# KrishnaswamyLab/MELD

Hardware: AMD Instinct MI355X
Metric: cells/sec through MELD.fit_transform (kNN+Chebyshev) (higher is better)
Workload: dtype f64

## Files before the change

### meld_amd/csrc/knn16.hip

```cpp
#include "common.hpp"
#include "k16_rows.hpp"

#include <hip/hip_fp16.h>

#include <algorithm>

namespace meld {

constexpr int K16_TS = 64;
constexpr int K16_BQ = 256;
constexpr int K16_THREADS = 256;
constexpr int K16_NWAVE = K16_THREADS / 64;
constexpr int K16_SLACK = 128;
constexpr int K16_CAPMAX = K16_ROW_CAPMAX;
constexpr int K16_BOUNDS_THREADS = 1024;
constexpr int K16_SLOTS = K16_CAPMAX / 64;
constexpr int K16_DMAX = 16 * 9 - 3;

constexpr int K16_SPLIT_DA = 13;
__host__ __device__ inline void k16_slot(int c, int d, int dA, int* coord, int* piece) {
  *coord = -1;
  *piece = -1;
  if (dA == 0) {
    if (c < d) *coord = c;
// ... 523 lines not shown
#pragma unroll
      for (int kb = 0; kb < KB; ++kb) {
        __builtin_amdgcn_sched_group_barrier(0x008, 1, 0);
        __builtin_amdgcn_sched_group_barrier(0x002, VALU_PER_MFMA, 0);
        __builtin_amdgcn_sched_group_barrier(0x008, 1, 0);
        __builtin_amdgcn_sched_group_barrier(0x002, VALU_PER_MFMA, 0);
        if (kb + A_AHEAD < KB) __builtin_amdgcn_sched_group_barrier(0x100, 1, 0);
      }
    }
  };
  auto segment = [&](const _Float16* tile, int sub, f32x16& n0, f32x16& n1, const f32x16& c0, const f32x16& c1, int ref_base, bool issue,
                     bool fresh) __attribute__((always_inline)) {
    if (issue) mfma_block(tile, sub, n0, n1);
    float m0, m1;
    vote(c0, c1, m0, m1);
    if (issue) asm volatile("" : "+v"(m0), "+v"(m1));
    const bool hit = m0 < thrp[0] || m1 < thrp[1];
    if (issue) pipeline_order();
    if (fresh && __any(hit)) {
      unsigned t0s = tm_now();
      select(c0, c1, m0, m1, ref_base);
      if (STATS) {
        const unsigned d = tm_now() - t0s;
        tm_sel += d;
        tm_mark += d;
      }
    }
  };

  auto next_step = [&](int after, int par_, bool* live) __attribute__((always_inline)) {
    if (!my_lb) {
      *live = true;
      return after + 1;
    }
    unsigned long long any = lds_union(par_) & win_rem;
    if (__builtin_expect(any == 0, 0)) {
      while (any == 0 && win_base + 64 < n_scan) {
        load_window(win_base + 64);
        my_live = __ballot(win_lb <= wmax + prune_margin);
        if (lane == 0) lds_wlive[2][wave] = my_live;
        __syncthreads();
        any = lds_union(2) & win_rem;
        __syncthreads();
      }
      K16_COLD_REGION_END();
    }
    if (any == 0) {
      *live = false;
      return n_scan;
    }
    const int i = (int)__ffsll((long long)any) - 1;
    *live = (my_live >> i) & 1ull;
    win_rem &= ~((2ull << i) - 1ull);
    return win_base + i;
  };

  int n_done = 0;
  auto ee_tile = [&](const _Float16* tile_r, int t) __attribute__((always_inline)) {
    const f16x8* a8 = reinterpret_cast<const f16x8*>(tile_r) + jq;
    const f16x8 aA = a8[h * K16_TS], aB = a8[32 + h * K16_TS];
    const float tA0 = thrp[0] + ee_c[0], tA1 = thrp[1] + ee_c[1];
#pragma unroll
    for (int sub = 0; sub < 2; ++sub) {
#pragma unroll
      for (int r = 0; r < 16; ++r) accA0[r] = accA1[r] = 0.0f;
      accA0 = __builtin_amdgcn_mfma_f32_32x32x16_f16(sub ? aB : aA, bhi[0][0], accA0, 0, 0, 0);
      accA1 = __builtin_amdgcn_mfma_f32_32x32x16_f16(sub ? aB : aA, bhi[1][0], accA1, 0, 0, 0);
      if (__any(min16(accA0) < tA0 || min16(accA1) < tA1)) {
        const f16x8* as = a8 + sub * 32;
#pragma unroll
        for (int kb = 1; kb < KB; ++kb) {
          const f16x8 ahi = as[(kb * 2 + h) * K16_TS];
          accA0 = __builtin_amdgcn_mfma_f32_32x32x16_f16(ahi, bhi[0][kb], accA0, 0, 0, 0);
          accA1 = __builtin_amdgcn_mfma_f32_32x32x16_f16(ahi, bhi[1][kb], accA1, 0, 0, 0);
        }
        const float m0 = min16(accA0), m1 = min16(accA1);
        if (__any(m0 < thrp[0] || m1 < thrp[1])) {
          const unsigned t0s = tm_now();
          select(accA0, accA1, m0, m1, t * K16_TS + 32 * sub + 4 * h);
          if (STATS) {
            const unsigned dsel = tm_now() - t0s;
            tm_sel += dsel;
            tm_mark += dsel;
          }
        }
        ++st_go;
      }
    }
    ++n_done;
  };
  int s_cur = 0;
  int par = 0;
  int it = 0;
  bool live_cur = true;
  bool pend = false;
  unsigned e_pref = 0u;
  int t_cur = tile_of(0);
  bool live_next = true;
  int s_next = next_step(0, 0, &live_next);
  int t_next = s_next < n_scan ? tile_of(s_next) : t_cur;
  if constexpr (LIST) {
    const unsigned e0 = list_entry(0), e1 = list_entry(1);
    e_pref = list_entry(2);
    t_cur = (int)(e0 & 0xFFFFFFu);
    live_cur = entry_live(e0);
    s_next = 1;
    t_next = s_next < n_scan ? (int)(e1 & 0xFFFFFFu) : t_cur;
    live_next = entry_live(e1);
  }
  if constexpr (!PAIR) {
    if (s_next < n_scan) {
      K16_LOAD(__builtin_amdgcn_readfirstlane(t_next), (unsigned)TILE_LDS_BYTES);
      K16_STAGED_BUT_LAST();
    } else {
      K16_STAGED();
    }
    K16_TILE_BARRIER();
  }
  unsigned rd_b = 0u, nx_b = (unsigned)TILE_LDS_BYTES, wr_b = 2u * (unsigned)TILE_LDS_BYTES;
  auto scan_step = [&]() __attribute__((always_inline)) {
    const int t = t_cur;
    const _Float16* tile_r = reinterpret_cast<const _Float16*>(reinterpret_cast<const char*>(lds_ring) + rd_b);
    const bool tm_live = live_cur;
    unsigned e_far = 0u;
    if constexpr (LIST) e_far = list_entry(s_next + 2);
    if (EE && live_cur) {
      ee_tile(tile_r, t);
    } else if (live_cur) {
      segment(tile_r, 0, accA0, accA1, accB0, accB1, refB, true, pend);
      segment(tile_r, 1, accB0, accB1, accA0, accA1, t * K16_TS + 4 * h, true, true);
      refB = t * K16_TS + 32 + 4 * h;
      pend = true;
      ++n_done;
    } else if (pend) {
      segment(nullptr, 0, accA0, accA1, accB0, accB1, refB, false, true);
      pend = false;
    }

    if (tm_live) tm_lap(tm_seg); else tm_lap(tm_idle);
    if (batch_every > 0 && (it & (batch_every - 1)) == batch_every - 1) {
      const int limit = ksel + K16_COLD(batch_slack);
      unsigned long long todo = 0;
#pragma unroll
      for (int g = 0; g < 2; ++g) {
        const int cg = g ? cnt[1] : cnt[0];
        const int tot = cg + __shfl_xor(cg, 32, 64);
        todo |= (__ballot(tot > limit) & 0xffffffffull) << (32 * g);
      }
      if (todo) {
        while (todo) {
          const int j = __ffsll((long long)todo) - 1;
          todo &= todo - 1;
          squeeze(j >> 5, j & 31);
          if (STATS) ++st_sq;
        }
        refresh_wmax();
        K16_COLD_REGION_END();
      }
    }

    bool live_nn = true;
    int s_nn, t_nn;
    if constexpr (LIST) {
      s_nn = min(s_next + 1, n_scan);
      t_nn = s_nn < n_scan ? (int)(e_pref & 0xFFFFFFu) : t_next;
      live_nn = entry_live(e_pref);
      e_pref = e_far;
    } else {
      s_nn = s_next < n_scan ? next_step(s_next, par, &live_nn) : n_scan;
      t_nn = s_nn < n_scan ? tile_of(s_nn) : t_next;
    }

    if (s_nn < n_scan) {
      K16_LOAD(__builtin_amdgcn_readfirstlane(t_nn), wr_b);
      tm_lap(tm_tail);
      K16_STAGED_BUT_LAST();
    } else {
      tm_lap(tm_tail);
      K16_STAGED();
    }
    tm_lap(tm_dma);
    if (my_lb) {
      my_live = __ballot(win_lb <= wmax + prune_margin);
      if (lane == 0) lds_wlive[par ^ 1][wave] = my_live;
    }
    tm_lap(tm_tail);
    K16_TILE_BARRIER();
    tm_lap(tm_bar);
    s_cur = s_next;
    t_cur = t_next;
    live_cur = live_next;
    s_next = s_nn;
    t_next = t_nn;
    live_next = live_nn;
    par ^= 1;
    ++it;
    const unsigned free_b = rd_b;
    rd_b = nx_b;
    nx_b = wr_b;
    wr_b = free_b;
  };
  tm_mark = tm_now();
  if constexpr (PAIR) {
    constexpr unsigned PB = 2u * (unsigned)TILE_LDS_BYTES;
    const int n_pairs = (n_scan + 1) >> 1;
    unsigned c0 = list_entry(0), c1 = list_entry(1), x0 = list_entry(2), x1 = list_entry(3);
    if (n_scan > 0) K16_LOAD(__builtin_amdgcn_readfirstlane((int)(c0 & 0xFFFFFFu)), 0u);
    if (n_scan > 1) K16_LOAD(__builtin_amdgcn_readfirstlane((int)(c1 & 0xFFFFFFu)), (unsigned)TILE_LDS_BYTES);
    K16_STAGED();
    K16_TILE_BARRIER();
    for (int p = 0; p < n_pairs; ++p) {
      const unsigned buf = (p & 1) ? PB : 0u, other = PB - buf;
      const unsigned f0 = list_entry(2 * p + 4), f1 = list_entry(2 * p + 5);
      if (2 * p + 2 < n_scan) K16_LOAD(__builtin_amdgcn_readfirstlane((int)(x0 & 0xFFFFFFu)), other);
      if (2 * p + 3 < n_scan) K16_LOAD(__builtin_amdgcn_readfirstlane((int)(x1 & 0xFFFFFFu)), other + (unsigned)TILE_LDS_BYTES);
      tm_lap(tm_tail);
      const char* ring = reinterpret_cast<const char*>(lds_ring);
      const bool live0 = entry_live(c0), live1 = 2 * p + 1 < n_scan && entry_live(c1);
      if (live0) ee_tile(reinterpret_cast<const _Float16*>(ring + buf), (int)(c0 & 0xFFFFFFu));
      if (live1) ee_tile(reinterpret_cast<const _Float16*>(ring + buf + TILE_LDS_BYTES), (int)(c1 & 0xFFFFFFu));
      if (live0 || live1) tm_lap(tm_seg); else tm_lap(tm_idle);
      if (batch_every > 0 && (p & (batch_every / 2 - 1)) == batch_every / 2 - 1) {
        const int limit = ksel + K16_COLD(batch_slack);
        unsigned long long todo = 0;
#pragma unroll
        for (int g = 0; g < 2; ++g) {
          const int cg = g ? cnt[1] : cnt[0];
          const int tot = cg + __shfl_xor(cg, 32, 64);
          todo |= (__ballot(tot > limit) & 0xffffffffull) << (32 * g);
        }
        while (todo) {
          const int j = __ffsll((long long)todo) - 1;
          todo &= todo - 1;
          squeeze(j >> 5, j & 31);
          if (STATS) ++st_sq;
        }
      }
      tm_lap(tm_tail);
      K16_STAGED();
      tm_lap(tm_dma);
      K16_TILE_BARRIER();
      tm_lap(tm_bar);
      c0 = x0;
      c1 = x1;
      x0 = f0;
      x1 = f1;
      ++it;
    }
  }
  while (!PAIR && s_cur < n_scan) scan_step();
  if (pend) segment(nullptr, 0, accA0, accA1, accB0, accB1, refB, false, true);
  {
    unsigned long long* tiles_done = K16_COLD(tiles_done);
    if (tiles_done && lane == 0) {
      atomicAdd(tiles_done, (unsigned long long)n_done);
      if (EE && K16_COLD(count_go)) atomicAdd(tiles_done + 1, (unsigned long long)st_go);
    }
  }

  unsigned long long* stats = STATS ? K16_COLD(stats) : nullptr;
  if (STATS && stats) {
    unsigned a = st_app;
#pragma unroll
    for (int off = 32; off > 0; off >>= 1) a += __shfl_xor(a, off, 64);
    if (lane == 0) {
      atomicAdd(stats + 0, (unsigned long long)(2 * n_done));
      atomicAdd(stats + 1, (unsigned long long)st_slow);
      atomicAdd(stats + 2, (unsigned long long)a);
      atomicAdd(stats + 3, (unsigned long long)st_sq);
      const int it_tiles = PAIR ? n_scan : it;
      if (wave == 0) atomicAdd(stats + 4, (unsigned long long)it_tiles);
      atomicAdd(stats + 5, (unsigned long long)tm_seg);
      atomicAdd(stats + 6, (unsigned long long)tm_sel);
      atomicAdd(stats + 7, (unsigned long long)tm_tail);
      atomicAdd(stats + 8, (unsigned long long)tm_dma);
      atomicAdd(stats + 9, (unsigned long long)tm_bar);
      atomicAdd(stats + 10, (unsigned long long)tm_idle);
      atomicAdd(stats + 11, (unsigned long long)it_tiles);
      if (EE) atomicAdd(stats + 12, (unsigned long long)st_go);
    }
  }
  const float out_scale = K16_COLD(scale_info)[1];
  float* cand_thr = K16_COLD(cand_thr);
  int* cand_cnt = K16_COLD(cand_cnt);
  if (cand_thr && h == 0) {
    cand_thr[row_base + jq] = (thrp[0] + wave_qn[jq]) * out_scale;
    cand_thr[row_base + 32 + jq] = (thrp[1] + wave_qn[32 + jq]) * out_scale;
  }
  {
    const int o0 = __shfl_xor(cnt[0], 32, 64), o1 = __shfl_xor(cnt[1], 32, 64);
    if (h == 0) {
      cand_cnt[row_base + jq] = cnt[0] | (o0 << 16);
      cand_cnt[row_base + 32 + jq] = cnt[1] | (o1 << 16);
    }
  }
#undef K16_LOAD
#undef K16_DMA
#undef K16_STAGED
#undef K16_STAGED_BUT_LAST
#undef K16_TILE_BARRIER
#undef K16_ROUND_OK
}

template <int TPS, int WPE>
__global__ __launch_bounds__(256) __attribute__((amdgpu_waves_per_eu(WPE, WPE))) void knn16_partial_filter_kernel(const _Float16* __restrict__ Q16, const float* __restrict__ Qn,
                                                                   const _Float16* __restrict__ Rt16, const float* __restrict__ scale_info,
                                                                   const float* __restrict__ norm2_max, const float* __restrict__ thr_init,
                                                                   unsigned* step_list, const int* __restrict__ step_cnt, long long list_stride,
                                                                   int* __restrict__ cnt_out, unsigned long long* __restrict__ tested,
                                                                   const int* __restrict__ block_order, int KB, int ee_hi) {
  static_assert(TPS >= 2 && TPS <= 32 && (TPS & 1) == 0, "tiles per step");
  __shared__ __attribute__((aligned(16))) _Float16 ring[2][TPS][2 * K16_TS * 8];
  __shared__ unsigned wmask[2][4];
  const int tid = threadIdx.x, lane = tid & 63;
  const int wave = __builtin_amdgcn_readfirstlane(tid >> 6);
  const int jq = lane & 31, h = lane >> 5;
  const int bx = block_order ? __builtin_amdgcn_readfirstlane(block_order[blockIdx.x]) : (int)blockIdx.x;
  const int q_base = bx * K16_BQ + wave * 64;
  f16x8 b0[2];
  float tA[2];
  {
    const float s_ = scale_info[0];
    const float delta = 3.814697265625e-06f * (norm2_max[0] * s_ * s_) + 1e-30f;
#pragma unroll
    for (int g = 0; g < 2; ++g) {
      const int q = q_base + g * 32 + jq;
      const f16x8* qrow = reinterpret_cast<const f16x8*>(Q16 + (size_t)q * (size_t)(KB * 32));
      b0[g] = qrow[h * 2];
      float qb = 0.0f;
      for (int kb = 1; kb < KB; ++kb) {
        const f16x8 v8 = qrow[(kb * 2 + h) * 2];
#pragma unroll
        for (int e = 0; e < 8; ++e) {
          const float v = (16 * kb + 8 * h + e < ee_hi) ? (float)v8[e] : 0.0f;
          qb = fmaf(v, v, qb);
        }
      }
      qb += __shfl_xor(qb, 32, 64);
      tA[g] = (thr_init[q] - Qn[q]) + (qb * 1.0001f + delta);
    }
  }
  unsigned* const my_list_w = step_list + (size_t)bx * (size_t)list_stride;
  const int n = __builtin_amdgcn_readfirstlane(step_cnt[bx]);
  const int n_steps = (n + TPS - 1) / TPS;
  const size_t tile_bytes = (size_t)KB * 4096;
  const int plane_stride = 2048;
  const size_t src_base = reinterpret_cast<size_t>(Rt16);
  typedef __attribute__((address_space(3))) void* lds_ptr_t;
  typedef int i32x4 __attribute__((ext_vector_type(4)));
  const unsigned ring_base = (unsigned)(size_t)(lds_ptr_t)&ring[0][0][0];
  const int lane16 = lane * 16;
  auto load_entries = [&](int step) __attribute__((always_inline)) {
    const int idx = step * TPS + lane;
    return (lane < TPS && idx < n) ? my_list_w[idx] : 0u;
  };
  auto stage = [&](unsigned ev, int buf) __attribute__((always_inline)) {
#pragma unroll
    for (int u = 0; u < TPS / 2; ++u) {
      const int k = wave * (TPS / 2) + u;
      const unsigned e = (unsigned)__builtin_amdgcn_readlane((int)ev, k >> 1);
      if (e >> 24) {
        const size_t src = src_base + (size_t)(e & 0xFFFFFFu) * tile_bytes;
        const i32x4 rsrc = {(int)(unsigned)src, (int)((src >> 32) & 0xffffu), 4096, 0x00020000};
        asm volatile("s_mov_b32 m0, %0\n\ts_nop 0\n\tbuffer_load_dwordx4 %1, %2, %3 offen lds" ::"s"(__builtin_amdgcn_readfirstlane(
                         (int)(ring_base + (unsigned)((buf * TPS + (k >> 1)) * 2048 + (k & 1) * 1024)))),
                     "v"(lane16), "s"(rsrc), "s"((k & 1) * plane_stride)
                     : "memory");
      }
    }
  };
  int out_n = 0;
  unsigned long long n_tested = 0;
  auto emit = [&](unsigned ev, int par) __attribute__((always_inline)) {
    unsigned nm = 0u;
#pragma unroll
    for (int w = 0; w < 4; ++w) nm |= ((wmask[par][w] >> lane) & 1u) << w;
    nm &= (ev >> 24);
    const bool keep = nm != 0u;
    const unsigned long long b = __ballot(keep);
    if (keep) my_list_w[out_n + __popcll(b & ((1ull << lane) - 1ull))] = (ev & 0xFFFFFFu) | (nm << 24);
    out_n += __popcll(b);
  };
  unsigned ev_prev = 0u, ev_cur = load_entries(0), ev_nxt = load_entries(1);
  if (n_steps > 0) stage(ev_cur, 0);
  __builtin_amdgcn_s_waitcnt(0x0F70);
  asm volatile("s_waitcnt lgkmcnt(0)\n\ts_barrier" ::: "memory");
  for (int s = 0; s < n_steps; ++s) {
    const int buf = s & 1;
    const unsigned ev_nn = load_entries(s + 2);
    if (s + 1 < n_steps) stage(ev_nxt, buf ^ 1);
    if (wave == 0 && s > 0) emit(ev_prev, buf ^ 1);
    unsigned mybits = 0u;
#pragma unroll
    for (int j = 0; j < TPS; ++j) {
      const unsigned e = (unsigned)__builtin_amdgcn_readlane((int)ev_cur, j);
      if ((e >> (24 + wave)) & 1u) {
        const f16x8* a8 = reinterpret_cast<const f16x8*>(&ring[buf][j][0]) + jq;
        const f16x8 aA = a8[h * K16_TS], aB = a8[h * K16_TS + 32];
        f32x16 c00, c01, c10, c11;
#pragma unroll
        for (int r = 0; r < 16; ++r) c00[r] = c01[r] = c10[r] = c11[r] = 0.0f;
        c00 = __builtin_amdgcn_mfma_f32_32x32x16_f16(aA, b0[0], c00, 0, 0, 0);
        c01 = __builtin_amdgcn_mfma_f32_32x32x16_f16(aA, b0[1], c01, 0, 0, 0);
        c10 = __builtin_amdgcn_mfma_f32_32x32x16_f16(aB, b0[0], c10, 0, 0, 0);
        c11 = __builtin_amdgcn_mfma_f32_32x32x16_f16(aB, b0[1], c11, 0, 0, 0);
        const bool hit = __builtin_fminf(min16(c00), min16(c10)) < tA[0] || __builtin_fminf(min16(c01), min16(c11)) < tA[1];
        if (__any(hit)) mybits |= 1u << j;
        ++n_tested;
      }
    }
    if (lane == 0) wmask[buf][wave] = mybits;
    __builtin_amdgcn_s_waitcnt(0x0F70);
    asm volatile("s_waitcnt lgkmcnt(0)\n\ts_barrier" ::: "memory");
    ev_prev = ev_cur;
    ev_cur = ev_nxt;
    ev_nxt = ev_nn;
  }
  if (wave == 0) {
    if (n_steps > 0) emit(ev_prev, (n_steps - 1) & 1);
    if (lane == 0) cnt_out[bx] = out_n;
  }
  if (tested && lane == 0) atomicAdd(tested, n_tested);
}

template <int SL>
__device__ __forceinline__ void k16_finish_row(float* __restrict__ drow, int* __restrict__ irow, int n0, int half, int n_all, int n,
                                               float add, float out_scale, int lane) {
  unsigned long long key[SL];
#pragma unroll
  for (int e = 0; e < SL; ++e) {
    const int i = lane + 64 * e;
    const int p = i < n0 ? i : half + (i - n0);
    key[e] = ~0ull;
    if (i < n_all) key[e] = ((unsigned long long)ordered_bits((drow[p] + add) * out_scale + 0.0f) << 32) | (unsigned)irow[p];
  }
  k16_bitonic_sort<SL>(key, lane);
#pragma unroll
  for (int e = 0; e < SL; ++e) {
    const int i = 64 * e + lane;
    if (i < n) {
      drow[i] = from_ordered_bits((unsigned)(key[e] >> 32));
      irow[i] = (int)(unsigned)key[e];
    }
  }
}
__global__ __launch_bounds__(256) void knn16_finish_rows_kernel(float* __restrict__ d2, int* __restrict__ idx,
                                                                int* __restrict__ cnt, const float* __restrict__ Qn,
                                                                const float* __restrict__ scale_info, int64_t n_rows,
                                                                int64_t q_pad, int cap, int ksel) {
  const int lane = threadIdx.x & 63;
  const int64_t row = (int64_t)blockIdx.x * 4 + (threadIdx.x >> 6);
  if (row >= n_rows) return;
  const int packed = cnt[row];
  const int n0 = packed & 0xffff, n1 = (packed >> 16) & 0xffff, half = cap >> 1;
  float* drow = d2 + (size_t)row * cap;
  int* irow = idx + (size_t)row * cap;
  const int n_all = n0 + n1, n = min(n_all, ksel);
  const float add = Qn[row % q_pad], out_scale = scale_info[1];
  if (n_all <= 64)
    k16_finish_row<1>(drow, irow, n0, half, n_all, n, add, out_scale, lane);
  else if (n_all <= 128)
    k16_finish_row<2>(drow, irow, n0, half, n_all, n, add, out_scale, lane);
  else
    k16_finish_row<K16_SLOTS>(drow, irow, n0, half, n_all, n, add, out_scale, lane);
  if (lane == 0) cnt[row] = n;
}

constexpr int K16_MERGE_MAX = 4096;
constexpr int K16_MERGE_SLOTS = K16_MERGE_MAX / 64;

__global__ __launch_bounds__(64) void knn16_merge_slices_kernel(const int* __restrict__ s_idx,
                                                                const float* __restrict__ s_d2,
                                                                const int* __restrict__ s_cnt, int q_count, int q_pad,
                                                                int ksel, int cap, int n_slices,
                                                                int* __restrict__ out_idx, float* __restrict__ out_d2,
                                                                int* __restrict__ out_cnt) {
  extern __shared__ __attribute__((aligned(16))) unsigned char merge_lds[];
  float* sd = reinterpret_cast<float*>(merge_lds);
  int* si = reinterpret_cast<int*>(merge_lds) + n_slices * ksel;
  const int lane = threadIdx.x;
  const int q = blockIdx.x;
  if (q >= q_count) return;
  int n = 0;
  for (int s = 0; s < n_slices; ++s) {
    const int row = s * q_pad + q;
    const int c = min(s_cnt[row], ksel);
    for (int e = lane; e < c; e += 64) {
      sd[n + e] = s_d2[(size_t)row * cap + e];
      si[n + e] = s_idx[(size_t)row * cap + e];
    }
    n += c;
  }
  __syncthreads();
  for (int p = lane; p < n; p += 64) {
    const float dp = sd[p];
    const int ip = si[p];
    int rk = 0;
    for (int e = 0; e < n; ++e) rk += (sd[e] < dp || (sd[e] == dp && si[e] < ip)) ? 1 : 0;
    if (rk < ksel) {
      out_d2[(size_t)q * cap + rk] = dp;
      out_idx[(size_t)q * cap + rk] = ip;
    }
  }
  if (lane == 0) out_cnt[q] = min(n, ksel);
}

__device__ __forceinline__ void k16_tile_sphere(const float* xs_dyn, int ld, int cnt, int d, int KB, int dA, int tile,
                                                _Float16* __restrict__ cent16, float* __restrict__ cent_n, float* __restrict__ cent_r) {
#define XS(r, k) xs_dyn[(r) * ld + (k)]
  __shared__ float cs[K16_DMAX + 19];
  const int tid = threadIdx.x;
  if (tid < KB * 16) {
    float acc = 0.0f;
    if (tid < d)
      for (int r = 0; r < cnt; ++r) acc += XS(r, tid);
    cs[tid] = tid < d ? acc / (float)cnt : 0.0f;
  }
  __syncthreads();
  __shared__ float cb[K16_DMAX + 19];
  __shared__ float s_best_r2;
  if (tid < 64) {
    const int lane = tid;
    auto far2 = [&](int* who) {
      float r2 = -1.0f;
      if (lane < cnt) {
        r2 = 0.0f;
        int k = 0;
        for (; k + 8 <= d; k += 8) {
          float t[8];
#pragma unroll
          for (int u = 0; u < 8; ++u) t[u] = XS(lane, k + u) - cs[k + u];
#pragma unroll
          for (int u = 0; u < 8; ++u) r2 = fmaf(t[u], t[u], r2);
        }
        for (; k < d; ++k) {
          const float t = XS(lane, k) - cs[k];
          r2 = fmaf(t, t, r2);
        }
      }
      auto dppf = [](float old, float v, auto ctrl, auto rows) __attribute__((always_inline)) {
        return __int_as_float(__builtin_amdgcn_update_dpp(__float_as_int(old), __float_as_int(v), decltype(ctrl)::value, decltype(rows)::value, 0xF, false));
      };
      using std::integral_constant;
      float m = r2;
      m = fmaxf(m, dppf(m, m, integral_constant<int, 0xB1>{}, integral_constant<int, 0xF>{}));
      m = fmaxf(m, dppf(m, m, integral_constant<int, 0x4E>{}, integral_constant<int, 0xF>{}));
      m = fmaxf(m, dppf(m, m, integral_constant<int, 0x141>{}, integral_constant<int, 0xF>{}));
      m = fmaxf(m, dppf(m, m, integral_constant<int, 0x140>{}, integral_constant<int, 0xF>{}));
      m = fmaxf(m, dppf(m, m, integral_constant<int, 0x142>{}, integral_constant<int, 0xA>{}));
      m = fmaxf(m, dppf(m, m, integral_constant<int, 0x143>{}, integral_constant<int, 0xC>{}));
      m = __int_as_float(__builtin_amdgcn_readlane(__float_as_int(m), 63));
      *who = __ffsll((long long)__ballot(r2 == m)) - 1;
      return m;
    };
    float best = INFINITY;
    constexpr int MEB_STEPS = 24;
    for (int it = 1; it <= MEB_STEPS + 1; ++it) {
      int who;
      const float r2 = far2(&who);
      if (r2 < best) {
        best = r2;
        for (int k = lane; k < KB * 16; k += 64) cb[k] = cs[k];
      }
      if (it <= MEB_STEPS) {
        const float wgt = 1.0f / (float)(it + 1);
        for (int k = lane; k < d; k += 64) cs[k] = fmaf(wgt, XS(who, k) - cs[k], cs[k]);
      }
      __builtin_amdgcn_s_waitcnt(0xC07F);
      asm volatile("" ::: "memory");
    }
    for (int k = lane; k < KB * 16; k += 64) cs[k] = cb[k];
    if (lane == 0) s_best_r2 = best;
  }
  __syncthreads();
  if (tid < 64) {
    const float r2 = s_best_r2;
    float n = 0.0f;
    for (int k = 0; k < d; ++k) n = fmaf(cs[k], cs[k], n);
    if (tid == 0) {
      cent_r[tile] = sqrtf(r2) * 1.0001f + 1e-30f;
      cent_n[tile] = n;
    }
  } else if (tid - 64 < KB * 2) {
    const int g = tid - 64;
    f16x8 hi, lo;
#pragma unroll
    for (int e = 0; e < 8; ++e) {
      int cc, pc;
      k16_slot(g * 8 + e, d, dA, &cc, &pc);
      _Float16 h16 = (_Float16)0.0f, l16 = (_Float16)0.0f;
      if (cc >= 0) {
        h16 = (_Float16)cs[cc];
        l16 = (_Float16)(cs[cc] - (float)h16);
      } else if (pc >= 0) {
        h16 = (_Float16)1.0f;
      }
      hi[e] = h16;
      lo[e] = l16;
    }
    f16x8* qrow = reinterpret_cast<f16x8*>(cent16) + (size_t)tile * ((size_t)KB * 4);
    qrow[g * 2 + 0] = hi;
    qrow[g * 2 + 1] = lo;
  }
#undef XS
}

__global__ __launch_bounds__(256) void tile_spheres_kernel(const double* __restrict__ X, int64_t N, int d,
                                                           const double* __restrict__ mean,
                                                           const float* __restrict__ scale_info, int KB,
                                                           _Float16* __restrict__ cent16, float* __restrict__ cent_n,
                                                           float* __restrict__ cent_r, int tile0, int dA) {
  extern __shared__ float xs_dyn[];
  const int ld = d | 1;
  const int tid = threadIdx.x;
  const int tile = tile0 + (int)blockIdx.x;
  const int64_t row0 = (int64_t)tile * K16_TS;
  const int cnt = (int)min((int64_t)K16_TS, N - row0);
  const float s = scale_info[0];
  for (int u = tid; u < K16_TS * d; u += 256) {
    const int r = u / d, k = u - r * d;
    const int64_t i = row0 + r;
    xs_dyn[r * ld + k] = i < N ? s * (float)(X[i * d + k] - mean[k]) : 0.0f;
  }
  __syncthreads();
  k16_tile_sphere(xs_dyn, ld, cnt, d, KB, dA, tile, cent16, cent_n, cent_r);
}

template <int KB, bool SEEDED, int BT, bool BITS = false, int KU = KB>
__global__ __launch_bounds__(BT) void knn16_tile_bounds_kernel(const _Float16* __restrict__ C16, const float* __restrict__ Cn,
                                                                const float* __restrict__ Cr,
                                                                const _Float16* __restrict__ Rt16, int n_tiles,
                                                                int first_tile, int n_blocks, float err_coef,
                                                                const float* __restrict__ norm2_max,
                                                                const float* __restrict__ scale_info,
                                                                const float* __restrict__ thr_seed, int64_t n_seed,
                                                                float seed_err_coef, int mark_sign,
                                                                const float* __restrict__ q_norm2, float err_c, float err_l,
                                                                __half* __restrict__ lb2, const float* __restrict__ wthr = nullptr,
                                                                unsigned long long* __restrict__ bits_a = nullptr,
                                                                unsigned long long* __restrict__ bits_b = nullptr, int wpr = 0, int dA = 0) {
  constexpr int TPB = 1;
  constexpr int HV = KU * 2 * K16_TS;
  constexpr int NS = (HV + BT - 1) / BT;
  __shared__ __attribute__((aligned(16))) float4 lds_a[2][HV];
  __shared__ __attribute__((aligned(16))) f16x8 lds_x[2][2 * K16_TS];
  const int tid = threadIdx.x, lane = tid & 63, wave = tid >> 6, jq = lane & 31, h = lane >> 5;
  const int c_base = blockIdx.x * BT + wave * 64;
  f16x8 bhi[2][KU];
  float cn[2], cr[2];
#pragma unroll
  for (int g = 0; g < 2; ++g) {
    const f16x8* qrow = reinterpret_cast<const f16x8*>(C16 + (size_t)(c_base + g * 32 + jq) * (KB * 32));
#pragma unroll
    for (int kb = 0; kb < KU; ++kb) bhi[g][kb] = qrow[(kb * 2 + h) * 2 + 0];
    cn[g] = Cn[c_base + g * 32 + jq];
    cr[g] = Cr[c_base + g * 32 + jq];
    if (KU < KB) {
      const f16x8 lo = qrow[(0 * 2 + h) * 2 + 1];
      float n = 0.0f;
#pragma unroll
      for (int e = 0; e < 8; ++e) {
        const float v = (8 * h + e < dA) ? (float)bhi[g][0][e] + (float)lo[e] : 0.0f;
        n = fmaf(v, v, n);
      }
      cn[g] = n + __shfl_xor(n, 32, 64);
    }
  }
  float wcol[2] = {-INFINITY, -INFINITY};
  if (BITS) {
#pragma unroll
    for (int g = 0; g < 2; ++g)
      if (c_base + g * 32 + jq < n_tiles) wcol[g] = wthr[c_base + g * 32 + jq];
  }
  const int c_l = c_base + lane;
  const float cn_l = h == 0 ? cn[0] : cn[1], cr_l = h == 0 ? cr[0] : cr[1], wcol_l = h == 0 ? wcol[0] : wcol[1];
  f16x8 bx[2];
#pragma unroll
  for (int g = 0; g < 2; ++g) {
#pragma unroll
    for (int e = 0; e < 8; ++e) bx[g][e] = (_Float16)0.0f;
    if (h == 0) {
      bx[g][0] = (_Float16)(-1.0f);
      bx[g][1] = (_Float16)(-__half2float(__float2half_ru(2.0f * cr[g])));
    }
  }
  const float err_abs = (err_coef + (KU < KB ? 1.9073486328125e-06f : 0.0f)) * norm2_max[0] * scale_info[0] * scale_info[0];
  const int b_lo = (int)((long long)n_blocks * blockIdx.y / gridDim.y);
  const int b_hi = (int)((long long)n_blocks * (blockIdx.y + 1) / gridDim.y);
  const int n_steps = (b_hi - b_lo) * TPB;
  const float4* R4 = reinterpret_cast<const float4*>(Rt16);
  float4 p[NS];
  float seed_v = 0.0f;
  const float nmax_s = norm2_max[0] * scale_info[0] * scale_info[0];
  const float seed_margin = seed_err_coef * nmax_s;
  float seed_nq = -1.0f;
  auto load = [&](int step) __attribute__((always_inline)) {
    const int t = first_tile + (b_lo * TPB + step);
#pragma unroll
    for (int u = 0; u < NS; ++u) {
      const int j = tid + BT * u;
      if (j < HV) p[u] = t < n_tiles ? R4[(size_t)t * (KB * 256) + ((j >> 6) << 7) + (j & 63)] : make_float4(0.f, 0.f, 0.f, 0.f);
    }
    if (SEEDED && tid < K16_TS) {
      const int64_t q = (int64_t)(b_lo * TPB + step) * K16_TS + tid;
      seed_v = q < n_seed ? thr_seed[q] : -1.0f;
      seed_nq = (q_norm2 != nullptr && q < n_seed) ? q_norm2[q] : -1.0f;
    }
  };
  auto store = [&](int buf) __attribute__((always_inline)) {
#pragma unroll
    for (int u = 0; u < NS; ++u) {
// ... 1018 lines not shown
    K16_BITS_CASE(7)
    K16_BITS_CASE(8)
    K16_BITS_CASE(9)
    default:
      set_err("meld_knn16_step_lists_direct: no kernel for %d K blocks", KB);
      return MELD_ERR_UNSUPPORTED;
  }
#undef K16_BITS_CASE
#undef K16_BITS_LAUNCH
  MELD_LAUNCH_CHECK("knn16_tile_bounds_kernel(bits)");
  const int64_t n_tiles64 = (int64_t)ceil_div(n_q, 64) * wpr;
  hipLaunchKernelGGL(knn16_bits_transpose_and_kernel, dim3((unsigned)ceil_div(n_tiles64, 4)), dim3(256), 0, st, bits_a, bits_b, n_q, wpr, live);
  hipLaunchKernelGGL(knn16_step_list_bits_kernel, dim3((unsigned)ceil_div(N, K16_BQ)), dim3(256), 0, st, live, wpr, n_t, 0, 1, list,
                     (long long)list_stride, cnt);
  MELD_LAUNCH_CHECK("knn16_step_list_bits_kernel");
  return MELD_OK;
}

extern "C" int meld_knn16_step_lists_direct(const double* X, int64_t N, int d, const double* mean, const float* scale_info,
                                            const float* norm2_max, const void* Rt16, const float* thr_seed, const float* q_norm2,
                                            int nprod, void* temp, void* scratch, uint32_t* list, int64_t list_stride, int32_t* cnt,
                                            meld_stream_t stream) {
  return k16_step_lists_direct_impl(X, N, d, mean, scale_info, norm2_max, Rt16, thr_seed, q_norm2, nprod, temp, scratch, list, list_stride, cnt, 0,
                                    stream);
}
extern "C" int meld_knn16_step_lists_direct_lead(const double* X, int64_t N, int d, const double* mean, const float* scale_info,
                                                 const float* norm2_max, const void* Rt16, const float* thr_seed, const float* q_norm2,
                                                 int nprod, void* temp, void* scratch, uint32_t* list, int64_t list_stride, int32_t* cnt,
                                                 int lead_only, meld_stream_t stream) {
  return k16_step_lists_direct_impl(X, N, d, mean, scale_info, norm2_max, Rt16, thr_seed, q_norm2, nprod, temp, scratch, list, list_stride, cnt,
                                    lead_only, stream);
}

extern "C" int meld_knn16_step_lists_direct_spheres(const double* X, int64_t N, int d, const double* mean, const float* scale_info,
                                                    const float* norm2_max, const void* Rt16, const float* thr_seed, const float* q_norm2,
                                                    int nprod, void* temp, void* scratch, uint32_t* list, int64_t list_stride, int32_t* cnt,
                                                    int lead_only, meld_stream_t stream) {
  return k16_step_lists_direct_impl(X, N, d, mean, scale_info, norm2_max, Rt16, thr_seed, q_norm2, nprod, temp, scratch, list, list_stride, cnt,
                                    lead_only, stream, true);
}

extern "C" int meld_knn16_seed_thresholds_mfma(const void* Q16, const float* Qn, const void* Rt16, const float* scale_info,
                                               const float* norm2_max, int64_t n_ref, int d, int64_t q_begin,
                                               int64_t q_count, int knn, double radius_factor, int nprod, int side_tiles,
                                               float* thr_init, meld_stream_t stream) {
  const int side = side_tiles > 0 ? side_tiles : (int)std::min<double>(64.0, std::max<double>(8.0, (double)n_ref / 12500.0));
  MELD_CHECK_ARG(Q16 && Qn && Rt16 && scale_info && norm2_max && thr_init && n_ref > 0 && q_count > 0 && q_begin >= 0,
                 "meld_knn16_seed_thresholds_mfma: bad arguments");
  MELD_CHECK_ARG(q_begin % K16_BQ == 0, "meld_knn16_seed_thresholds_mfma: q_begin must be a multiple of the query block (%d)", K16_BQ);
  MELD_CHECK_ARG(knn >= 1 && radius_factor >= 1.0 && (nprod == 1 || nprod == 3), "meld_knn16_seed_thresholds_mfma: bad kernel parameters");
  const int KB = meld_knn16_kblocks(d);
  if (KB < 0) return KB;
  const int n_b = (int)ceil_div(q_count, K16_BQ);
  hipStream_t st = S(stream);
  if (knn + 1 > SEED_KMAX) {
    MELD_HIP_CALL(hipMemsetD32Async(reinterpret_cast<hipDeviceptr_t>(thr_init), 0x7f800000, (size_t)n_b * K16_BQ, st));
    return MELD_OK;
  }
  const float rf2 = (float)(radius_factor * radius_factor * (1.0 + 1e-6));
  const int n_tiles = (int)ceil_div(n_ref, K16_TS);
  const float ec = (float)meld_knn16_error_coef_const(1, d), el = (float)meld_knn16_error_coef_lin(1);
  (void)nprod;
#define K16_SEEDM_LAUNCH(KBV, KV)                                                                                       \
  hipLaunchKernelGGL((knn16_seed_mfma_kernel<KBV, KV>), dim3((unsigned)ceil_div(n_b * K16_NWAVE, SEED_WAVES)),            \
                     dim3(64 * SEED_WAVES), 0, st, reinterpret_cast<const _Float16*>(Q16), Qn,                            \
                     reinterpret_cast<const _Float16*>(Rt16), scale_info, norm2_max, n_tiles, (int)(q_begin / K16_TS),   \
                     side, n_b * K16_NWAVE, knn + 1, rf2, ec, el, thr_init)
#define K16_SEEDM_CASE(KBV)          \
  case KBV:                          \
    if (knn + 1 <= 16)               \
      K16_SEEDM_LAUNCH(KBV, 16);     \
    else                             \
      K16_SEEDM_LAUNCH(KBV, 64);     \
    break;
  switch (KB) {
    K16_SEEDM_CASE(1)
    K16_SEEDM_CASE(2)
    K16_SEEDM_CASE(3)
    K16_SEEDM_CASE(4)
    K16_SEEDM_CASE(5)
    K16_SEEDM_CASE(6)
    K16_SEEDM_CASE(7)
    K16_SEEDM_CASE(8)
    K16_SEEDM_CASE(9)
    default:
      set_err("meld_knn16_seed_thresholds_mfma: no kernel for %d K blocks", KB);
      return MELD_ERR_UNSUPPORTED;
  }
#undef K16_SEEDM_CASE
#undef K16_SEEDM_LAUNCH
  MELD_LAUNCH_CHECK("knn16_seed_mfma_kernel");
  return MELD_OK;
}

template <int KB, int STATS>
static void k16_launch_topk(dim3 grid, hipStream_t st, const K16Args& ka, bool listed, bool ee, int nprod) {
  if (listed) {
    if constexpr (KB >= 2 && KB <= 7) {
      if (ee) {
        hipLaunchKernelGGL((knn16_topk_kernel<KB, STATS, 1, true, true>), grid, dim3(K16_THREADS), 0, st, ka);
        return;
      }
    }
    hipLaunchKernelGGL((knn16_topk_kernel<KB, STATS, 1, true>), grid, dim3(K16_THREADS), 0, st, ka);
  } else if (nprod == 1) {
    hipLaunchKernelGGL((knn16_topk_kernel<KB, STATS, 1>), grid, dim3(K16_THREADS), 0, st, ka);
  } else {
    hipLaunchKernelGGL((knn16_topk_kernel<KB, STATS, 3>), grid, dim3(K16_THREADS), 0, st, ka);
  }
}

static int k16_topk_impl(const void* Q16, const float* Qn, const void* Rt16, const float* scale_info,
                         int64_t n_ref, int d,
                         int64_t q_count, int ksel, int nprod, int n_slices, const void* lb2,
                         const float* norm2_max, int64_t q_begin, const float* thr_init, int knn,
                         double radius_factor, int32_t* cand_idx, float* cand_d2, int32_t* cand_cnt,
                         float* cand_thr, uint64_t* tiles_done, const int32_t* block_order, const uint32_t* step_list,
                         const int32_t* step_cnt, int64_t list_stride, meld_stream_t stream, int partial_test = 0, int two_counters = 0,
                         bool finish = true) {
  MELD_CHECK_ARG(nprod == 1 || nprod == 3, "meld_knn16_topk: nprod must be 1 or 3");
  MELD_CHECK_ARG(finish || n_slices == 1, "meld_knn16_topk_listed_raw: raw rows go with one slice (the merge of slices takes finished rows)");
  MELD_CHECK_ARG(step_list == nullptr || (step_cnt != nullptr && nprod == 1 && lb2 == nullptr && thr_init != nullptr),
                 "meld_knn16_topk_listed: step lists go with the hi-only pass, start thresholds and no table");
  MELD_CHECK_ARG(n_slices >= 1 && n_slices * ksel <= K16_MERGE_MAX, "meld_knn16_topk: n_slices=%d must satisfy n_slices * ksel <= %d",
                 n_slices, K16_MERGE_MAX);
  MELD_CHECK_ARG(Q16 && Qn && Rt16 && scale_info && cand_idx && cand_d2 && cand_cnt, "meld_knn16_topk: null pointer");
  MELD_CHECK_ARG(lb2 == nullptr || norm2_max != nullptr, "meld_knn16_topk: pruning needs norm2_max");
  MELD_CHECK_ARG(cand_thr == nullptr || (norm2_max != nullptr && knn >= 0 && knn < ksel && radius_factor >= 1.0),
                 "meld_knn16_topk: the radius cut needs norm2_max, 0 <= knn < ksel, radius_factor >= 1");
  const int knn1 = (cand_thr && knn >= 1) ? knn + 1 : 0;
  const float rf2 = knn1 > 0 ? (float)(radius_factor * radius_factor * (1.0 + 1e-6)) : 0.0f;
  const float err_c = (float)meld_knn16_error_coef_const(nprod, d), err_l = (float)meld_knn16_error_coef_lin(nprod);
  MELD_CHECK_ARG(n_ref > 0 && n_ref < (int64_t)1 << 31 && q_count > 0, "meld_knn16_topk: bad sizes");
  const int cap = meld_knn16_row_capacity(ksel);
  if (cap < 0) return cap;
  const int KB = meld_knn16_kblocks(d);
  if (KB < 0) return KB;
  const int n_tiles = (int)ceil_div(n_ref, K16_TS);
  const dim3 grid((unsigned)n_slices, (unsigned)ceil_div(q_count, K16_BQ));
  MELD_CHECK_ARG(grid.y <= 65535u, "meld_knn16_topk: more than 65535 query blocks in one launch");
  MELD_CHECK_ARG(n_slices <= ceil_div(n_ref, K16_TS), "meld_knn16_topk: more slices than reference tiles");
  const int tile_origin = (int)((q_begin / K16_TS) % n_tiles);
  const _Float16* q = reinterpret_cast<const _Float16*>(Q16);
  const _Float16* r = reinterpret_cast<const _Float16*>(Rt16);
  unsigned long long* stats = nullptr;
  if (meld_dev_getenv("MELD_KNN16_STATS")) {
    static unsigned long long* counters[64] = {nullptr};
    int dev = 0;
    MELD_HIP_CALL(hipGetDevice(&dev));
    MELD_CHECK_ARG(dev >= 0 && dev < 64, "meld_knn16_topk: device index out of range");
    if (counters[dev] == nullptr) MELD_HIP_CALL(hipMalloc(reinterpret_cast<void**>(&counters[dev]), 256));
    MELD_HIP_CALL(hipMemsetAsync(counters[dev], 0, 256, S(stream)));
    stats = counters[dev];
  }
  K16Args ka;
  ka.Q16 = q;
  ka.Qn = Qn;
  ka.Rt16 = r;
  ka.scale_info = scale_info;
  ka.n_ref = (int)n_ref;
  ka.n_tiles = n_tiles;
  ka.ksel = ksel;
  ka.cap = cap;
  ka.lb2 = reinterpret_cast<const __half*>(lb2);
  ka.norm2_max = norm2_max;
  ka.err_coef = (float)meld_knn16_error_coef(nprod, d);
  ka.tile_origin = tile_origin;
  ka.batch_every = 64;
  ka.batch_slack = 64;
  ka.two_sided = 1;
  ka.stats = stats;
  ka.thr_init = thr_init;
  ka.knn1 = knn1;
  ka.rf2 = rf2;
  ka.err_c = err_c;
  ka.err_l = err_l;
  ka.cand_idx = cand_idx;
  ka.cand_d2 = cand_d2;
  ka.cand_cnt = cand_cnt;
  ka.cand_thr = cand_thr;
  ka.tiles_done = reinterpret_cast<unsigned long long*>(tiles_done);
  ka.block_order = block_order;
  ka.step_list = step_list;
  ka.step_cnt = step_cnt;
  ka.list_stride = (long long)list_stride;
  const int dA = k16_dA(d, KB);
  const bool ee = step_list != nullptr && dA > 0 && KB >= 2 && KB <= 7 && partial_test != 0;
  ka.ee_hi = 16 + d - dA;
  ka.count_go = two_counters;
  ka.planes_used = ((dA > 0 ? 16 + (d - dA) + 3 : d + 3) + 7) / 8;
#define K16_CASE(KBV)                                                                                                      \
  case KBV:                                                                                                                \
    (stats ? k16_launch_topk<KBV, 1> : k16_launch_topk<KBV, 0>)(grid, S(stream), ka, step_list != nullptr, ee, nprod); \
    break;
  switch (KB) {
    K16_CASE(1)
    K16_CASE(2)
    K16_CASE(3)
    K16_CASE(4)
    K16_CASE(5)
    K16_CASE(6)
    K16_CASE(7)
    K16_CASE(8)
    K16_CASE(9)
    default:
      set_err("meld_knn16_topk: KB=%d is not an instantiated size", KB);
      return MELD_ERR_UNSUPPORTED;
  }
#undef K16_CASE
  MELD_LAUNCH_CHECK("knn16_topk_kernel");
  if (finish) {
    const int64_t n_rows = (int64_t)grid.x * K16_BQ * grid.y;
    hipLaunchKernelGGL(knn16_finish_rows_kernel, dim3((unsigned)ceil_div(n_rows, 4)), dim3(256), 0, S(stream), cand_d2, cand_idx, cand_cnt, Qn,
                       scale_info, n_rows, (int64_t)grid.y * K16_BQ, cap, ksel);
    MELD_LAUNCH_CHECK("knn16_finish_rows_kernel");
  }
  if (stats) {
    unsigned long long st[13] = {0, 0, 0, 0, 0, 0, 0, 0, 0, 0, 0, 0, 0};
    MELD_HIP_CALL(hipStreamSynchronize(S(stream)));
    MELD_HIP_CALL(hipMemcpy(st, stats, sizeof(st), hipMemcpyDeviceToHost));
    fprintf(stderr, "[knn16 stats] wave-blocks %llu  slow-path entries %llu (%.1f %%)  appends %llu (%.1f per query)  compactions %llu  tiles staged %llu (%.1f %% of workgroups x tiles)\n",
            st[0], st[1], st[0] ? 100.0 * (double)st[1] / (double)st[0] : 0.0, st[2], (double)st[2] / (double)q_count, st[3], st[4],
            100.0 * (double)st[4] / ((double)grid.y * (double)n_tiles));
    if (ee)
      fprintf(stderr, "[knn16 stats] blocks of 32 references that went on past K block 0: %llu of %llu (%.1f %%)\n", st[12], st[0],
              st[0] ? 100.0 * (double)st[12] / (double)st[0] : 0.0);
    {
      const double tot = (double)(st[5] + st[6] + st[7] + st[8] + st[9] + st[10]);
      fprintf(stderr, "[knn16 stats] wave cycles (s_memtime units, summed over waves; %% of the scan loop): MFMA segments of live steps %.1f  slow path %.1f  "
                      "control tail %.1f  tile wait %.1f  barrier %.1f  steps sat out %.1f   -- per wave and staged tile: %.0f units; live wave-steps %.1f %%\n",
              100.0 * st[5] / tot, 100.0 * st[6] / tot, 100.0 * st[7] / tot, 100.0 * st[8] / tot, 100.0 * st[9] / tot, 100.0 * st[10] / tot,
              tot / (double)st[11], st[11] ? 50.0 * (double)st[0] / (double)st[11] : 0.0);
    }
  }
  return MELD_OK;
}

extern "C" int meld_knn16_topk(const void* Q16, const float* Qn, const void* Rt16, const float* scale_info,
                               int64_t n_ref, int d,
                               int64_t q_count, int ksel, int nprod, int n_slices, const void* lb2,
                               const float* norm2_max, int64_t q_begin, const float* thr_init, int knn,
                               double radius_factor, int32_t* cand_idx, float* cand_d2, int32_t* cand_cnt,
                               float* cand_thr, uint64_t* tiles_done, const int32_t* block_order, meld_stream_t stream) {
  return k16_topk_impl(Q16, Qn, Rt16, scale_info, n_ref, d, q_count, ksel, nprod, n_slices, lb2, norm2_max, q_begin, thr_init, knn,
                       radius_factor, cand_idx, cand_d2, cand_cnt, cand_thr, tiles_done, block_order, nullptr, nullptr, 0, stream);
}

extern "C" int meld_knn16_topk_listed(const void* Q16, const float* Qn, const void* Rt16, const float* scale_info, int64_t n_ref,
                                      int d, int64_t q_count, int ksel, const uint32_t* step_list, const int32_t* step_cnt,
                                      int64_t list_stride, const float* norm2_max, int64_t q_begin, const float* thr_init, int knn,
                                      double radius_factor, int32_t* cand_idx, float* cand_d2, int32_t* cand_cnt, float* cand_thr,
                                      uint64_t* tiles_done, const int32_t* block_order, int n_slices, meld_stream_t stream) {
  MELD_CHECK_ARG(step_list && step_cnt && list_stride > 0, "meld_knn16_topk_listed: null step lists");
  return k16_topk_impl(Q16, Qn, Rt16, scale_info, n_ref, d, q_count, ksel, 1, n_slices, nullptr, norm2_max, q_begin, thr_init, knn,
                       radius_factor, cand_idx, cand_d2, cand_cnt, cand_thr, tiles_done, block_order, step_list, step_cnt, list_stride,
                       stream);
}

extern "C" int meld_knn16_topk_listed_partial(const void* Q16, const float* Qn, const void* Rt16, const float* scale_info, int64_t n_ref,
                                              int d, int64_t q_count, int ksel, const uint32_t* step_list, const int32_t* step_cnt,
                                              int64_t list_stride, const float* norm2_max, int64_t q_begin, const float* thr_init, int knn,
                                              double radius_factor, int32_t* cand_idx, float* cand_d2, int32_t* cand_cnt, float* cand_thr,
                                              uint64_t* tiles_done, const int32_t* block_order, int n_slices, int partial_test,
                                              meld_stream_t stream) {
  MELD_CHECK_ARG(step_list && step_cnt && list_stride > 0, "meld_knn16_topk_listed_partial: null step lists");
  return k16_topk_impl(Q16, Qn, Rt16, scale_info, n_ref, d, q_count, ksel, 1, n_slices, nullptr, norm2_max, q_begin, thr_init, knn,
                       radius_factor, cand_idx, cand_d2, cand_cnt, cand_thr, tiles_done, block_order, step_list, step_cnt, list_stride,
                       stream, partial_test, 1);
}

extern "C" int meld_knn16_topk_listed_raw(const void* Q16, const float* Qn, const void* Rt16, const float* scale_info, int64_t n_ref,
                                          int d, int64_t q_count, int ksel, const uint32_t* step_list, const int32_t* step_cnt,
                                          int64_t list_stride, const float* norm2_max, int64_t q_begin, const float* thr_init, int knn,
                                          double radius_factor, int32_t* cand_idx, float* cand_d2, int32_t* cand_cnt, float* cand_thr,
                                          uint64_t* tiles_done, const int32_t* block_order, int partial_test, meld_stream_t stream) {
  MELD_CHECK_ARG(step_list && step_cnt && list_stride > 0, "meld_knn16_topk_listed_raw: null step lists");
  return k16_topk_impl(Q16, Qn, Rt16, scale_info, n_ref, d, q_count, ksel, 1, 1, nullptr, norm2_max, q_begin, thr_init, knn,
                       radius_factor, cand_idx, cand_d2, cand_cnt, cand_thr, tiles_done, block_order, step_list, step_cnt, list_stride,
                       stream, partial_test, 1, false);
}

extern "C" int meld_knn16_finish_rows(float* cand_d2, int32_t* cand_idx, int32_t* cand_cnt, const float* Qn, const float* scale_info,
                                      int64_t n_rows, int ksel, meld_stream_t stream) {
  MELD_CHECK_ARG(cand_d2 && cand_idx && cand_cnt && Qn && scale_info && n_rows > 0, "meld_knn16_finish_rows: bad arguments");
  const int cap = meld_knn16_row_capacity(ksel);
  if (cap < 0) return cap;
  hipLaunchKernelGGL(knn16_finish_rows_kernel, dim3((unsigned)ceil_div(n_rows, 4)), dim3(256), 0, S(stream), cand_d2, cand_idx, cand_cnt, Qn,
                     scale_info, n_rows, n_rows, cap, ksel);
  MELD_LAUNCH_CHECK("knn16_finish_rows_kernel");
  return MELD_OK;
}

extern "C" int meld_knn16_partial_filter(const void* Q16, const float* Qn, const void* Rt16, const float* scale_info, const float* norm2_max,
                                         int d, int64_t q_count, const float* thr_init, uint32_t* step_list, const int32_t* step_cnt,
                                         int64_t list_stride, int32_t* cnt_out, uint64_t* tested, const int32_t* block_order,
                                         meld_stream_t stream) {
  MELD_CHECK_ARG(Q16 && Qn && Rt16 && scale_info && norm2_max && thr_init && step_list && step_cnt && cnt_out && list_stride > 0 && q_count > 0,
                 "meld_knn16_partial_filter: null pointer or bad sizes");
  const int KB = meld_knn16_kblocks(d);
  if (KB < 0) return KB;
  const int dA = k16_dA(d, KB);
  MELD_CHECK_ARG(dA > 0 && KB >= 2, "meld_knn16_partial_filter: d = %d has no split operand layout", d);
  const unsigned n_blocks = (unsigned)ceil_div(q_count, K16_BQ);
  hipLaunchKernelGGL((knn16_partial_filter_kernel<8, 4>), dim3(n_blocks), dim3(256), 0, S(stream), reinterpret_cast<const _Float16*>(Q16), Qn,
                     reinterpret_cast<const _Float16*>(Rt16), scale_info, norm2_max, thr_init, step_list, step_cnt, (long long)list_stride, cnt_out,
                     reinterpret_cast<unsigned long long*>(tested), block_order, KB, 16 + d - dA);
  MELD_LAUNCH_CHECK("knn16_partial_filter_kernel");
  return MELD_OK;
}

extern "C" int meld_knn16_resident_blocks(int d, int nprod) {
  MELD_CHECK_ARG(nprod == 1 || nprod == 3, "meld_knn16_resident_blocks: nprod must be 1 or 3");
  const int KB = meld_knn16_kblocks(d);
  if (KB < 0) return KB;
  int per_cu = 0;
#define K16_OCC(KBV)                                                                                              \
  case KBV:                                                                                                       \
    if (nprod == 1) {                                                                                             \
      MELD_HIP_CALL(hipOccupancyMaxActiveBlocksPerMultiprocessor(&per_cu, knn16_topk_kernel<KBV, 0, 1>, K16_THREADS, 0)); \
    } else {                                                                                                      \
      MELD_HIP_CALL(hipOccupancyMaxActiveBlocksPerMultiprocessor(&per_cu, knn16_topk_kernel<KBV, 0, 3>, K16_THREADS, 0)); \
    }                                                                                                             \
    break;
  switch (KB) {
    K16_OCC(1)
    K16_OCC(2)
    K16_OCC(3)
    K16_OCC(4)
    K16_OCC(5)
    K16_OCC(6)
    K16_OCC(7)
    K16_OCC(8)
    K16_OCC(9)
    default:
      return MELD_ERR_UNSUPPORTED;
  }
#undef K16_OCC
  int dev = 0, cus = 0;
  MELD_HIP_CALL(hipGetDevice(&dev));
  MELD_HIP_CALL(hipDeviceGetAttribute(&cus, hipDeviceAttributeMultiprocessorCount, dev));
  return per_cu * cus;
}

extern "C" int meld_knn16_max_slices(int ksel) { return ksel < 1 ? MELD_ERR_INVALID : std::max(1, K16_MERGE_MAX / ksel); }

extern "C" int meld_knn16_merge_slices(const int32_t* s_idx, const float* s_d2, const int32_t* s_cnt, int64_t q_count,
                                       int ksel, int n_slices, int32_t* out_idx, float* out_d2, int32_t* out_cnt,
                                       meld_stream_t stream) {
  MELD_CHECK_ARG(s_idx && s_d2 && s_cnt && out_idx && out_d2 && out_cnt && q_count > 0, "meld_knn16_merge_slices: null");
  const int cap = meld_knn16_row_capacity(ksel);
  if (cap < 0) return cap;
  MELD_CHECK_ARG(n_slices >= 1 && n_slices * ksel <= K16_MERGE_MAX, "meld_knn16_merge_slices: too many slices");
  const int q_pad = (int)(ceil_div(q_count, K16_BQ) * K16_BQ);
  hipLaunchKernelGGL(knn16_merge_slices_kernel, dim3((unsigned)q_count), dim3(64), (size_t)n_slices * ksel * 8, S(stream), s_idx, s_d2,
                     s_cnt, (int)q_count, q_pad, ksel, cap, n_slices, out_idx, out_d2, out_cnt);
  MELD_LAUNCH_CHECK("knn16_merge_slices_kernel");
  return MELD_OK;
}
```

Measured before the change: 29.14 million.

## Restructure kNN filter: single buffer descriptor, per-wave tile staging, early-exit second MFMA

Tile staging now gives each wave a contiguous group of tiles and loads both planes of a tile itself. When the reference set fits in 4 GiB, it uses one buffer descriptor over the whole set plus a scalar offset, so no per-tile descriptor is built. The filter loop walks only live tiles via a ballot mask and software-pipelines the fragment loads and MFMAs. It skips the second query group's MFMAs when the first group already hits, which saves matrix work on hit-heavy tiles. This adds control-flow complexity and uses list_stride as the tile count when sizing the descriptor, which assumes that bound holds.

```diff
diff --git a/meld_amd/csrc/knn16.hip b/meld_amd/csrc/knn16.hip
--- a/meld_amd/csrc/knn16.hip
+++ b/meld_amd/csrc/knn16.hip
@@ -849,14 +849,14 @@
 #undef K16_ROUND_OK
 }
 
-template <int TPS, int WPE>
+template <int TPS, int WPE, bool ONE_DESC>
 __global__ __launch_bounds__(256) __attribute__((amdgpu_waves_per_eu(WPE, WPE))) void knn16_partial_filter_kernel(const _Float16* __restrict__ Q16, const float* __restrict__ Qn,
                                                                    const _Float16* __restrict__ Rt16, const float* __restrict__ scale_info,
                                                                    const float* __restrict__ norm2_max, const float* __restrict__ thr_init,
                                                                    unsigned* step_list, const int* __restrict__ step_cnt, long long list_stride,
                                                                    int* __restrict__ cnt_out, unsigned long long* __restrict__ tested,
-                                                                   const int* __restrict__ block_order, int KB, int ee_hi) {
-  static_assert(TPS >= 2 && TPS <= 32 && (TPS & 1) == 0, "tiles per step");
+                                                                   const int* __restrict__ block_order, int KB, int ee_hi, unsigned n_tiles) {
+  static_assert(TPS >= 4 && TPS <= 32 && (TPS & 3) == 0, "tiles per step");
   __shared__ __attribute__((aligned(16))) _Float16 ring[2][TPS][2 * K16_TS * 8];
   __shared__ unsigned wmask[2][4];
   const int tid = threadIdx.x, lane = tid & 63;
@@ -901,18 +901,33 @@
     const int idx = step * TPS + lane;
     return (lane < TPS && idx < n) ? my_list_w[idx] : 0u;
   };
+  const i32x4 rsrc_all = {(int)(unsigned)src_base, (int)((src_base >> 32) & 0xffffu), (int)(n_tiles * (unsigned)tile_bytes), 0x00020000};
+  const unsigned wave_ring = __builtin_amdgcn_readfirstlane((int)(ring_base + (unsigned)(wave * (TPS / 4) * 2048)));
   auto stage = [&](unsigned ev, int buf) __attribute__((always_inline)) {
-#pragma unroll
-    for (int u = 0; u < TPS / 2; ++u) {
-      const int k = wave * (TPS / 2) + u;
-      const unsigned e = (unsigned)__builtin_amdgcn_readlane((int)ev, k >> 1);
+    const unsigned dst = wave_ring + (unsigned)(buf * TPS * 2048);
+#pragma unroll
+    for (int u = 0; u < TPS / 4; ++u) {
+      const int slot = wave * (TPS / 4) + u;
+      const unsigned e = (unsigned)__builtin_amdgcn_readlane((int)ev, slot);
       if (e >> 24) {
-        const size_t src = src_base + (size_t)(e & 0xFFFFFFu) * tile_bytes;
-        const i32x4 rsrc = {(int)(unsigned)src, (int)((src >> 32) & 0xffffu), 4096, 0x00020000};
-        asm volatile("s_mov_b32 m0, %0\n\ts_nop 0\n\tbuffer_load_dwordx4 %1, %2, %3 offen lds" ::"s"(__builtin_amdgcn_readfirstlane(
-                         (int)(ring_base + (unsigned)((buf * TPS + (k >> 1)) * 2048 + (k & 1) * 1024)))),
-                     "v"(lane16), "s"(rsrc), "s"((k & 1) * plane_stride)
-                     : "memory");
+        if (ONE_DESC) {
+          const unsigned off = (e & 0xFFFFFFu) * (unsigned)tile_bytes;
+          asm volatile("s_add_u32 m0, %0, %4\n\ts_nop 0\n\tbuffer_load_dwordx4 %1, %2, %3 offen lds" ::"s"(dst), "v"(lane16), "s"(rsrc_all),
+                       "s"(off), "i"(u * 2048)
+                       : "memory", "scc");
+          asm volatile("s_add_u32 m0, %0, %4\n\ts_nop 0\n\tbuffer_load_dwordx4 %1, %2, %3 offen lds" ::"s"(dst), "v"(lane16), "s"(rsrc_all),
+                       "s"(off + (unsigned)plane_stride), "i"(u * 2048 + 1024)
+                       : "memory", "scc");
+        } else {
+          const size_t src = src_base + (size_t)(e & 0xFFFFFFu) * tile_bytes;
+          const i32x4 rsrc = {(int)(unsigned)src, (int)((src >> 32) & 0xffffu), 4096, 0x00020000};
+#pragma unroll
+          for (int pl = 0; pl < 2; ++pl)
+            asm volatile("s_mov_b32 m0, %0\n\ts_nop 0\n\tbuffer_load_dwordx4 %1, %2, %3 offen lds" ::"s"(__builtin_amdgcn_readfirstlane(
+                             (int)(dst + (unsigned)(u * 2048 + pl * 1024)))),
+                         "v"(lane16), "s"(rsrc), "s"(pl * plane_stride)
+                         : "memory");
+        }
       }
     }
   };
@@ -927,6 +942,22 @@
     const unsigned long long b = __ballot(keep);
     if (keep) my_list_w[out_n + __popcll(b & ((1ull << lane) - 1ull))] = (ev & 0xFFFFFFu) | (nm << 24);
     out_n += __popcll(b);
+  };
+  const unsigned frag_lane = (unsigned)((h * K16_TS + jq) * 16);
+  auto frags = [&](int buf, int j, f16x8& aA, f16x8& aB) __attribute__((always_inline)) {
+    const f16x8* a8 = reinterpret_cast<const f16x8*>(reinterpret_cast<const char*>(&ring[0][0][0]) + (unsigned)((buf * TPS + j) * 2048) + frag_lane);
+    aA = a8[0];
+    aB = a8[32];
+  };
+  auto group = [&](const f16x8& aA, const f16x8& aB, const f16x8& b, f32x16& cA, f32x16& cB) __attribute__((always_inline)) {
+    f32x16 z;
+#pragma unroll
+    for (int r = 0; r < 16; ++r) z[r] = 0.0f;
+    cA = __builtin_amdgcn_mfma_f32_32x32x16_f16(aA, b, z, 0, 0, 0);
+    cB = __builtin_amdgcn_mfma_f32_32x32x16_f16(aB, b, z, 0, 0, 0);
+  };
+  auto below = [&](const f32x16& cA, const f32x16& cB, float t) __attribute__((always_inline)) {
+    return __ballot(__builtin_fminf(min16(cA), min16(cB)) < t);
   };
   unsigned ev_prev = 0u, ev_cur = load_entries(0), ev_nxt = load_entries(1);
   if (n_steps > 0) stage(ev_cur, 0);
@@ -938,22 +969,36 @@
     if (s + 1 < n_steps) stage(ev_nxt, buf ^ 1);
     if (wave == 0 && s > 0) emit(ev_prev, buf ^ 1);
     unsigned mybits = 0u;
-#pragma unroll
-    for (int j = 0; j < TPS; ++j) {
-      const unsigned e = (unsigned)__builtin_amdgcn_readlane((int)ev_cur, j);
-      if ((e >> (24 + wave)) & 1u) {
-        const f16x8* a8 = reinterpret_cast<const f16x8*>(&ring[buf][j][0]) + jq;
-        const f16x8 aA = a8[h * K16_TS], aB = a8[h * K16_TS + 32];
-        f32x16 c00, c01, c10, c11;
-#pragma unroll
-        for (int r = 0; r < 16; ++r) c00[r] = c01[r] = c10[r] = c11[r] = 0.0f;
-        c00 = __builtin_amdgcn_mfma_f32_32x32x16_f16(aA, b0[0], c00, 0, 0, 0);
-        c01 = __builtin_amdgcn_mfma_f32_32x32x16_f16(aA, b0[1], c01, 0, 0, 0);
-        c10 = __builtin_amdgcn_mfma_f32_32x32x16_f16(aB, b0[0], c10, 0, 0, 0);
-        c11 = __builtin_amdgcn_mfma_f32_32x32x16_f16(aB, b0[1], c11, 0, 0, 0);
-        const bool hit = __builtin_fminf(min16(c00), min16(c10)) < tA[0] || __builtin_fminf(min16(c01), min16(c11)) < tA[1];
-        if (__any(hit)) mybits |= 1u << j;
-        ++n_tested;
+    unsigned live = (unsigned)__ballot(((ev_cur >> (24 + wave)) & 1u) != 0u);
+    n_tested += (unsigned)__builtin_popcount(live);
+    if (live) {
+      int j = __builtin_ctz(live);
+      live &= live - 1u;
+      f16x8 a0A, a0B, a1A, a1B;
+      f32x16 xA, xB, yA, yB;
+      frags(buf, j, a0A, a0B);
+      group(a0A, a0B, b0[0], xA, xB);
+      auto pair = [&](const f16x8& cA, const f16x8& cB, f16x8& nA, f16x8& nB) __attribute__((always_inline)) {
+        const bool more = live != 0u;
+        const int jn = more ? __builtin_ctz(live) : j;
+        frags(buf, jn, nA, nB);
+        const unsigned long long m0 = below(xA, xB, tA[0]);
+        __builtin_amdgcn_sched_barrier(0);
+        if (more) group(nA, nB, b0[0], xA, xB);
+        __builtin_amdgcn_sched_barrier(0);
+        unsigned long long m1 = 0ull;
+        if (m0 == 0ull) {
+          group(cA, cB, b0[1], yA, yB);
+          m1 = below(yA, yB, tA[1]);
+        }
+        if ((m0 | m1) != 0ull) mybits |= 1u << j;
+        live &= live - 1u;
+        j = jn;
+        return more;
+      };
+      for (;;) {
+        if (!pair(a0A, a0B, a1A, a1B)) break;
+        if (!pair(a1A, a1B, a0A, a0B)) break;
       }
     }
     if (lane == 0) wmask[buf][wave] = mybits;
@@ -2578,9 +2623,14 @@
   const int dA = k16_dA(d, KB);
   MELD_CHECK_ARG(dA > 0 && KB >= 2, "meld_knn16_partial_filter: d = %d has no split operand layout", d);
   const unsigned n_blocks = (unsigned)ceil_div(q_count, K16_BQ);
-  hipLaunchKernelGGL((knn16_partial_filter_kernel<8, 4>), dim3(n_blocks), dim3(256), 0, S(stream), reinterpret_cast<const _Float16*>(Q16), Qn,
-                     reinterpret_cast<const _Float16*>(Rt16), scale_info, norm2_max, thr_init, step_list, step_cnt, (long long)list_stride, cnt_out,
-                     reinterpret_cast<unsigned long long*>(tested), block_order, KB, 16 + d - dA);
+  const unsigned long long rt_bytes = (unsigned long long)list_stride * (unsigned long long)KB * 4096ull;
+#define MELD_FILTER_LAUNCH(ONE)                                                                                                              \
+  hipLaunchKernelGGL((knn16_partial_filter_kernel<8, 4, ONE>), dim3(n_blocks), dim3(256), 0, S(stream), reinterpret_cast<const _Float16*>(Q16), Qn, \
+                     reinterpret_cast<const _Float16*>(Rt16), scale_info, norm2_max, thr_init, step_list, step_cnt, (long long)list_stride, cnt_out, \
+                     reinterpret_cast<unsigned long long*>(tested), block_order, KB, 16 + d - dA, (unsigned)(ONE ? list_stride : 0))
+  if (rt_bytes < (1ull << 32)) MELD_FILTER_LAUNCH(true);
+  else MELD_FILTER_LAUNCH(false);
+#undef MELD_FILTER_LAUNCH
   MELD_LAUNCH_CHECK("knn16_partial_filter_kernel");
   return MELD_OK;
 }
```

Measured after the change: 29.68 million, median of 6. About the same (+1.8%).
